# WasifurRahman/BERT_multimodal_transformer

Measured on AMD Instinct MI355X. Metric: train samples/sec MAG-BERT MOSI seq_len=50, higher is better.
Workload: dtype bf16; 1 GPU; MAG-BERT bert-base-uncased, MOSI dims (V=47, A=74), batch 48/GPU, seq_len 50, full optimizer step (fwd+MSE+bwd+HF-AdamW+schedule+zero_grad; inputs resident in HBM), dropout on, random-init weights; global_batch=48, seq_len=50, parallelism=dp1, step_call=mb_bert_train_step, hipGraph replay

## Files before the change

### bert_multimodal_transformer_amd/csrc/engine.hip

```cpp
#include "dp_step.h"

struct LayerOff { size_t wqkv, wo, w1, w2, bqkv, bo, ln1w, ln1b, b1, b2, ln2w, ln2b; };
struct LayerWs { size_t qkv, ctx, s1, st1, y1, u, g, s2, st2, stats; };

struct mb_bert_engine : StepMixin {
    mb_bert_config c;
    std::vector<TensorInfo> tensors;
    std::vector<LayerOff> lo;
    size_t word, pos, type, emb_lnw, emb_lnb, wp, bp, wc, bc;
    size_t mag_whv, mag_wha, mag_wv, mag_wa, mag_bhv, mag_bha, mag_bv, mag_ba, mag_lnw, mag_lnb;
    size_t n_params, n_decay, sh_begin, sh_end;
    size_t n_update_end() const { return n_params; }
    int n_layers() const { return c.num_layers; }
    size_t layer_begin(int l) const { return lo[l].wqkv; }
    size_t layers_end() const { return wp; }
    int width() const { return c.hidden_size; }
    size_t layer_end(int l) const { return l + 1 < c.num_layers ? lo[l + 1].wqkv : wp; }
    bool embed_all_frozen() const { return range_frozen(word, mag_whv) && range_frozen(emb_lnw, bp); }
    WordSkip word_skip(char* w) const {
        if (!(stamp_off != 0 && stamp_enable && idcnt_enable)) return {};
        return WordSkip{stamp_table(w), stamp_state(w), word, word + (size_t)c.vocab_size * c.hidden_size, (uint32_t)c.hidden_size};
    }
    MagWs mw;
    size_t ws_mag, ws_emb, ws_emb_st, ws_head_z, ws_head_pooled, ws_logits;
// ... 6 lines not shown
    size_t ws_ids, ws_seg, ws_mask, ws_labels;
    size_t ws_bytes;
    float* P = nullptr; float* G = nullptr; char* SH = nullptr; char* ws = nullptr;
    const int64_t* ids = nullptr; const int64_t* seg = nullptr; const int64_t* mask = nullptr;
    int B = 0, L = 0, training = 0;
    int padT = -1;
    int prefetch = 1;
    int pf_qkv = 0;
    RideOpts ride_opts;
    int ride_blocks = 0;
    float* ride_m = nullptr; float* ride_v = nullptr;
    size_t ride_cursor = 0;
    long ride_params = 0;
    int group_wgrad = 256;
    bool grouped = false;
    float* attn_out = nullptr;
    const float* head_mask = nullptr;
    const float* emb_in = nullptr;
    const int64_t* pos_ids = nullptr;
    bool ran_forward = false;

    bool ws_zeroed = false;
    uint64_t seed = 0, step = 0;
    float* logits = nullptr;

    size_t add(const std::string& name, std::vector<int64_t> shape, int decay, size_t& cursor) {
        TensorInfo t;
        t.name = name; t.ndim = (int)shape.size(); t.decay = decay; t.numel = 1;
        for (int i = 0; i < 4; ++i) t.shape[i] = i < t.ndim ? shape[i] : 1;
        for (auto s : shape) t.numel *= (size_t)s;
// ... 310 lines not shown
    if (!cfg || !out) return MB_ERR_ARG;
    const int Hc = cfg->hidden_size;
    if ((Hc != 256 && Hc != 512 && Hc != 768 && Hc != 1024) || cfg->num_heads * 64 != Hc || cfg->num_layers < 1) return MB_ERR_SHAPE;
    if (cfg->intermediate_size % 128 || cfg->max_seq < 1 || cfg->max_seq > 512 || cfg->max_batch < 1) return MB_ERR_SHAPE;
    if (cfg->max_seq > cfg->max_position || cfg->num_labels < 1) return MB_ERR_SHAPE;
    if (cfg->dtype != DT_F32 && cfg->dtype != DT_BF16) return MB_ERR_DTYPE;
    mb_bert_engine* e = new mb_bert_engine();
    e->c = *cfg;
    e->read_env();
    e->ride_opts.read_env();
    e->group_wgrad = env_int("MB_GROUP_WGRAD", e->group_wgrad);
    e->ride_blocks = env_int("MB_ADAMW_RIDE_BLOCKS", e->ride_blocks);
    e->ride_params = env_long("MB_ADAMW_RIDE_PARAMS", e->ride_params);
    e->prefetch = env_int("MB_PREFETCH", e->prefetch);
    e->pf_qkv = env_int("MB_PF_QKV", e->pf_qkv);
    if (e->group_wgrad == 256 && (cfg->dtype != DT_BF16 || cfg->hidden_size % 256 != 0 || cfg->intermediate_size % 256 != 0)) e->group_wgrad = 128;
    e->grouped = (e->group_wgrad == 64 || e->group_wgrad == 128 || e->group_wgrad == 256) && cfg->hidden_size % e->group_wgrad == 0 &&
                 cfg->intermediate_size % e->group_wgrad == 0;

    build_layout(e);
    e->ow_covers = e->grouped;
    e->stale_begin = e->lo[0].wqkv; e->stale_end = e->wp;
    *out = e;
    return MB_OK;
}
void mb_bert_destroy(mb_bert_engine* e) {
    if (!e) return;
    e->destroy_prof();
    e->drop_graphs();
    e->free_class_table();
// ... 134 lines not shown
        const bool sh_ok = e->c.dtype != DT_BF16 || (e->sh_begin <= rb && re <= e->sh_end);
        if (take == 0 || rb % 4 || !sh_ok) return r;
        const bool keep = e->keep_in_step() && e->stale_begin <= rb && re <= e->stale_end;
        r = AdamRide{e->P + rb, e->G + rb, e->ride_m + rb, e->ride_v + rb, e->c.dtype == DT_BF16 ? (bf16*)(e->SH + rb * 2) : nullptr,
                     take / 4, dyn, blocks / 8 * 8, keep ? 0 : 1};
        e->ride_cursor = rb;
        return r;
    };
    if (stage_begin < 0) stage_begin = 0;
    if (stage_end > NL + 2) stage_end = NL + 2;
    if (stage_begin == 0) CK(e->begin_backward_pass(e->G, st));
    float* P = e->P; float* G = e->G;
    char* ws = e->ws;
    const bool hd = e->training && c.hidden_dropout > 0.f;
    const GradAcc acc = e->acc_of(ws, G);
    for (int stage = stage_begin; stage < stage_end; ++stage) {
        if (stage == 0) {
            CK(head_backward(dt, dlogits, e->logits, labels, loss_scale, (const float*)(ws + e->ws_head_pooled), P + e->wc,
                             ws + e->ws_dz, G + e->wc, G + e->bc, B, H, c.num_labels, e->key(SITE_HEAD, c.hidden_dropout),
                             st, acc, G + e->bp, ws + e->ws_dxa, (size_t)T * H * esize(dt)));
            const char* xf = ws + e->ws_x[NL];
            CK(gemm(dt, GEMM_TN, EPI_ACCUM_F32, H, H, B, ws + e->ws_dz, H, xf, L * H, nullptr, H, nullptr, G + e->wp, nullptr,
                    nullptr, 0, kNoDrop, 1, 64, st));
            CK(gemm(dt, GEMM_NN, EPI_ADD_RES, B, H, H, ws + e->ws_dz, H, e->W(e->wp), H, ws + e->ws_dxa, L * H, nullptr,
                    nullptr, nullptr, nullptr, 0, kNoDrop, 1, 64, st));
        } else if (stage <= NL) {
            const int l = NL - stage;
            const LayerOff& o = e->lo[l];
            const LayerWs& w = e->lw[l];
            char* dx = ws + e->ws_dxa;
            char* dy1 = ws + e->ws_dxb;
            const int par = l & 1;
            char* dsA = ws + e->ws_ds[par];
            char* dzdA = hd ? ws + e->ws_dzd[par] : dsA;
            char* dsB = ws + e->ws_ds2[par];
            char* dzdB = hd ? ws + e->ws_dzd2[par] : dsB;
            char* du = ws + e->ws_du[par];
            char* dqkv = ws + e->ws_dqkv[par];
            int nblk = 0;
            float* lnp_a = (float*)(ws + e->ws_lnp_a) + (size_t)l * e->lnp_stride;
            float* lnp_b = (float*)(ws + e->ws_lnp_b) + (size_t)l * e->lnp_stride;
            const bool defer_ln = e->in_step && !e->stage_mode && NL + 2 <= MB_LN_MAX_LAYERS;
            CK(ln_backward_partials(dt, dx, ws + w.s2, P + o.ln2w, (const float*)(ws + w.st2), (const float*)(ws + w.st2) + T, dsA,
                                    hd ? dzdA : nullptr, lnp_a, &nblk, T, H, e->key(SITE_LAYER0 + 4 * l + 2, c.hidden_dropout), st,
                                    Prefetch{e->prefetch ? e->W(o.w1) : nullptr, (size_t)2 * I * H * (dt == DT_BF16 ? 2 : 4), nullptr}));
            GemmArgs wg[4] = {wgrad_args(H, I, Tk, dzdA, H, ws + w.g, I, G + o.w2, I),
                              wgrad_args(I, H, Tk, du, I, ws + w.y1, H, G + o.w1, H),
                              wgrad_args(H, H, Tk, dzdB, H, ws + w.ctx, H, G + o.wo, H),
                              wgrad_args(3 * H, H, Tk, dqkv, 3 * H, ws + e->ws_x[l], H, G + o.wqkv, H)};
            const bool grouped = e->grouped;
            const bool wfrozen = e->skipping() && e->unwritten(o.wqkv, e->layer_end(l));
            if (wfrozen) ++e->frz_wgrad_skipped;
            if (grouped)
                for (GemmArgs& a : wg) a.overwrite = e->ow_pass ? 1 : 0;
            auto dgrad_ride = [&](int mode, int Mo, int No, int Ko, const void* dY, int ldy, const void* Wt, int ldw, void* dX, int ldx, const void* R, int ldr,
                                  float* colsum) -> int {
                return dgrad_with_riders(dt, mode, Mo, No, Ko, dY, ldy, Wt, ldw, dX, ldx, R, ldr, colsum, kNoDrop, acc, st, grouped && e->ride_m != nullptr,
// ... 79 lines not shown
                                 G + e->emb_lnb, B, L, H, c.pad_token_id, e->key(SITE_EMB, c.hidden_dropout), st, e->pos_ids, acc,
                                 (float*)(ws + e->ws_lnp_a) + (size_t)(NL + 1) * e->lnp_stride, &eblk,
                                 (float*)(ws + e->ws_lnp_b) + (size_t)(NL + 1) * e->lnp_stride,
                                 (e->in_step && e->counted && e->ids && !e->emb_in) ? (int*)(ws + e->idcnt_off) : nullptr));
            {
                const int first = defer_ln ? 0 : NL;
                LnReduceDst dst = {};
                for (int k = first; k < NL; ++k) {
                    const LayerOff& ok = e->lo[k];
                    float* const d6[6] = {G + ok.ln2w, G + ok.ln2b, G + ok.b2, G + ok.ln1w, G + ok.ln1b, G + ok.bo};
                    for (int q = 0; q < 6; ++q) dst.d[k - first][q] = d6[q];
                }
                float* const m6[6] = {G + e->mag_bhv, G + e->mag_bha, G + e->mag_bv, G + e->mag_ba, G + e->mag_lnw, G + e->mag_lnb};
                for (int q = 0; q < 6; ++q) dst.d[NL - first][q] = m6[q];
                dst.nblk[NL - first] = mblk; dst.nblk[NL + 1 - first] = eblk;
                if (!emb_frozen) { dst.d[NL + 1 - first][0] = G + e->emb_lnw; dst.d[NL + 1 - first][1] = G + e->emb_lnb; }
                if (e->pos_ids == nullptr && !emb_frozen) {
                    dst.d[NL + 1 - first][2] = G + e->type; dst.d[NL + 1 - first][3] = G + e->type + H;
                }
                CK(ln_reduce_partials_layers((const float*)(ws + e->ws_lnp_a) + (size_t)first * e->lnp_stride,
                                             (const float*)(ws + e->ws_lnp_b) + (size_t)first * e->lnp_stride, e->lnp_stride, NL + 2 - first,
                                             e->lnp_nblk, H, dst, st, acc));
            }
            CK(grad_fold(acc, G, e->det_begin, e->det_end, st));
        }
    }
    return MB_OK;
}


static int enqueue_step(mb_bert_engine* e, int B, int L, float* logits, float* loss, float* loss_run, float* m, float* v,
                        float loss_scale, hipStream_t st) {
    char* ws = e->ws;
    const int NL = e->c.num_layers;
    const float* lab = (const float*)(ws + e->ws_in_lab);
    float* keep_attn = e->attn_out;
    e->attn_out = nullptr;
// ... 133 lines not shown
    e->attn_out = nullptr;
    struct Restore { mb_bert_engine* e; float* p; ~Restore() { e->attn_out = p; } } restore{e, keep_attn};
    return e->run_stage_graph(B, L, -1, 0, logits, loss, loss_run, 0.f, mode, st, [&](hipStream_t s) {
        return mb_bert_forward(e, (const int64_t*)(ws + e->ws_in_ids), (const float*)(ws + e->ws_in_vis), (const float*)(ws + e->ws_in_aco),
                               (const int64_t*)(ws + e->ws_in_mask), (const int64_t*)(ws + e->ws_in_seg), (const float*)(ws + e->ws_in_lab), B, L, 1,
                               0, 0, logits, loss, loss_run, s);
    });
}
int mb_bert_stage_backward(mb_bert_engine* e, float loss_scale, int stage, int mode, void* stream) {
    hipStream_t st = (hipStream_t)stream;
    if (!e || !e->G || !e->ran_forward || !e->training) return MB_ERR_ARG;
    if (stage < 0 || stage > e->c.num_layers + 1 || (mode != 1 && mode != 2)) return MB_ERR_ARG;
    if (e->prof) mode = 2;
    if (stage == 0) CK(e->begin_backward_pass(e->G, st));
    const float* lab = (const float*)(e->ws + e->ws_in_lab);
    return e->run_stage_graph(e->B, e->L, stage, e->ow_pass ? 1 : 0, e->logits, nullptr, nullptr, loss_scale, mode, st, [&](hipStream_t s) {
        return mb_bert_backward(e, nullptr, lab, loss_scale, stage, stage + 1, s);
    });
}

const int64_t* mb_bert_staged_input_ids(const mb_bert_engine* e) { return (e && e->ws) ? (const int64_t*)(e->ws + e->ws_in_ids) : nullptr; }

int mb_bert_load_batch(mb_bert_engine* e, const int64_t* input_ids, const float* visual, const float* acoustic,
                       const int64_t* attention_mask, const int64_t* token_type_ids, const float* labels, int B, int L,
                       const void** staged6, void* stream) {
    hipStream_t st = (hipStream_t)stream;
    if (!e || !e->ws || !staged6) return MB_ERR_ARG;
    const mb_bert_config& c = e->c;
    if (B < 1 || B > c.max_batch || L < 1 || L > c.max_seq) return MB_ERR_SHAPE;
    if (!input_ids || !visual || !acoustic || !attention_mask || !token_type_ids) return MB_ERR_ARG;
    const int T = B * L;
// ... 67 lines not shown
    return MB_OK;
}
int mb_bert_set_position_ids(mb_bert_engine* e, const int64_t* position_ids) {
    if (!e) return MB_ERR_ARG;
    e->pos_ids = position_ids;
    return MB_OK;
}
const float* mb_bert_inputs_embeds_grad(const mb_bert_engine* e) {
    if (!e || !e->ws || !e->ran_forward) return nullptr;
    return (const float*)(e->ws + e->ws_dsum);
}
int mb_bert_backward_outputs(mb_bert_engine* e, const void* d_sequence_output, const void* d_pooler_preact, void* stream) {
    hipStream_t st = (hipStream_t)stream;
    if (!e || !e->G || !e->ran_forward) return MB_ERR_ARG;
    CK(e->begin_backward_pass(e->G, st));
    const mb_bert_config& c = e->c;
    const int dt = c.dtype, H = c.hidden_size, B = e->B, L = e->L, T = B * L, NL = c.num_layers;
    char* ws = e->ws;
    const size_t bytes = (size_t)T * H * esize(dt);
    if (d_sequence_output) CK((int)hipMemcpyAsync(ws + e->ws_dxa, d_sequence_output, bytes, hipMemcpyDeviceToDevice, st));
    else CK(zero_fill(ws + e->ws_dxa, bytes, st));
    if (d_pooler_preact) {
        const char* xf = ws + e->ws_x[NL];
        CK(gemm(dt, GEMM_TN, EPI_ACCUM_F32, H, H, B, d_pooler_preact, H, xf, L * H, nullptr, H, nullptr, e->G + e->wp, nullptr, nullptr, 0,
                kNoDrop, 1, 64, st));
        CK(colsum(dt, d_pooler_preact, H, e->G + e->bp, B, H, st, e->acc_of(ws, e->G)));
        CK(gemm(dt, GEMM_NN, EPI_ADD_RES, B, H, H, d_pooler_preact, H, e->W(e->wp), H, ws + e->ws_dxa, L * H, nullptr, nullptr, nullptr,
                ws + e->ws_dxa, L * H, kNoDrop, 1, 64, st));
    }
    return MB_OK;
// ... 31 lines not shown
```

### bert_multimodal_transformer_amd/csrc/engine_common.h

```cpp
#pragma once
#include <string>
#include <vector>
#include <cstring>
#include <cstdio>
#include <cstdlib>
#include <cmath>
#include <algorithm>
#include "kernels.h"
#include "../../include/magbert_hip.h"

using namespace mb;
static_assert(MB_UPDATE_CLASSES_MAX == MB_CLASSES_MAX && MB_UPDATE_SEGMENTS_MAX == MB_SEGMENTS_MAX, "public limits = the kernels' limits");

namespace {

struct TensorInfo {
    std::string name;
    size_t off, numel;
    int ndim;
    int64_t shape[4];
    int decay;
};

inline size_t align_up(size_t x, size_t a) { return (x + a - 1) / a * a; }
// ... 222 lines not shown
            int dev = 0, n = 0;
            if (hipGetDevice(&dev) == hipSuccess && hipDeviceGetAttribute(&n, hipDeviceAttributeMultiprocessorCount, dev) == hipSuccess) cus = n;
            if (cus <= 0) cus = 256;
        }
        return cus;
    }
    bool grads_stale = false, ow_covers = false;
    size_t stale_begin = 0, stale_end = 0;
    int keep_enable = 1;
    bool keep_in_step() const { return keep_enable && ow_enable && ow_covers && stale_end > stale_begin; }
    int materialize_grads(float* G, hipStream_t st) {
        if (grads_stale && G) CK(zero_fill(G + stale_begin, (stale_end - stale_begin) * sizeof(float), st));
        grads_stale = false;
        return MB_OK;
    }
    int begin_backward_pass(float* G, hipStream_t st) {
        if (in_step) return MB_OK;
        stamp_live = word_zero = false;
        frz_dirty = true;
        ow_pass = grads_zero && ow_enable;
        grads_zero = false;
        if (!(ow_pass && ow_covers)) CK(materialize_grads(G, st));
        grads_stale = false;
        return MB_OK;
    }

    bool prof = false;
    std::vector<hipEvent_t> pev;
    int prof_layers = 0;
    int set_profiling(int on, int layers) {
        if (on && pev.empty()) {
// ... 583 lines not shown
```

### bert_multimodal_transformer_amd/csrc/gemm.hip

```cpp
#include "gemm_tile.h"
#include "adamw_dev.h"

namespace mb {

constexpr int PITCH = 144;

template <class T, int BROWS, bool KMAJ>
struct Stager {
    static constexpr int EPV = 16 / sizeof(T);
    static constexpr int BKE = 128 / sizeof(T);
    static constexpr int NREG = BROWS / 8;
    uint32_t r[NREG];

    __device__ __forceinline__ void load(const T* __restrict__ base, int ld, int row0, int nrows, int k0, int kend, int tid) {
        if constexpr (!KMAJ) {
#pragma unroll
            for (int i = 0; i < BROWS / 32; ++i) {
                const int rr = (tid >> 3) + 32 * i, c = tid & 7;
                const int g = row0 + rr;
                u32x4 v = {0u, 0u, 0u, 0u};
                if (g < nrows) v = *(const u32x4*)(base + (size_t)g * ld + k0 + c * EPV);
                r[4 * i + 0] = v[0]; r[4 * i + 1] = v[1]; r[4 * i + 2] = v[2]; r[4 * i + 3] = v[3];
            }
        } else {
// ... 593 lines not shown
        }
        return launch_cfg<T, 128, 128, AK, BK, MODE>(a, splits, st);
    } else
    if (v2ok) {
        int ns = 2, kb = 128;
        if (env.stages > 0) { kb = (env.stages / 10 == 2) ? 64 : 128; ns = env.stages % 10; }
        if (kb == 64 && (p.kchunk % (64 / (int)sizeof(T)) != 0)) kb = 128;
        if (sizeof(T) == 2 && ns <= 2 && p.kchunk / (kb / (int)sizeof(T)) < 2) ns = 3;
#define MB_LAUNCH2(NS, KBV) MB_GEMM_LAUNCH((gemm2_kernel<T, BM, BN, AK, BK, MODE, NS, KBV>), grid, dim3(256), st, p, &p, 1)
        if constexpr (BM == 64 && BN == 64 && sizeof(T) == 2) {
            if (env.ksplit && env.stages <= 0 && p.kchunk % 128 == 0 && p.kchunk >= 1024 && splits == 1 && tiles <= 512) {
                MB_GEMM_LAUNCH((gemm2_kernel<T, BM, BN, AK, BK, MODE, 2, 256, true>), grid, dim3(256), st, p, &p, 1);
                return (int)hipGetLastError();
            }
            if (env.stages64 >= 3 && env.stages <= 0 && splits == 1 && p.kchunk / BKE >= 2 && tiles <= 512) ns = env.stages64 > 4 ? 4 : env.stages64;
        }
        if (kb == 128) {
            if (BM == 128) { if (ns <= 2) MB_LAUNCH2(2, 128); else if (ns == 3) MB_LAUNCH2(3, 128); else MB_LAUNCH2(4, 128); }
            else { if (ns <= 2) MB_LAUNCH2(2, 128); else if (ns == 3) MB_LAUNCH2(3, 128); else MB_LAUNCH2(4, 128); }
        } else {
            if (ns <= 3) MB_LAUNCH2(3, 64); else if (ns == 4) MB_LAUNCH2(4, 64); else MB_LAUNCH2(5, 64);
        }
#undef MB_LAUNCH2
    } else {
        MB_GEMM_LAUNCH((gemm_kernel<T, BM, BN, AK, BK, MODE>), grid, dim3(256), st, p, &p, 1);
    }
    return (int)hipGetLastError();
}

static int tile_n768() { return host_env().tile_n768; }
// ... 242 lines not shown
```

### bert_multimodal_transformer_amd/csrc/gemm_tile.h

```cpp
#pragma once
#include <cstdlib>
#include <algorithm>
#include <type_traits>
#include "kernels.h"

namespace mb {

template <int BM, int BN>
__device__ __forceinline__ bool tile_origin(const GemmArgs& p, int& m0, int& n0, int bid = blockIdx.x) {
    const int xcd = bid & 7, j = bid >> 3;
    const int xm = xcd / p.reg_n, xn = xcd % p.reg_n;
    const int tm = xm * p.tpr_m + j / p.tpr_n, tn = xn * p.tpr_n + j % p.tpr_n;
    m0 = tm * BM;
    n0 = tn * BN;
    return m0 < p.M && n0 < p.N && (j / p.tpr_n) < p.tpr_m;
}

template <int BM, int BN>
__device__ __forceinline__ bool grouped_tile_origin(const GroupedGemmArgs& ga, int& g, int& m0, int& n0) {
    const int bid = (int)blockIdx.x - ga.ride.blocks;
    g = 0;
    if (ga.chunk > 0) {
        const int xcd = bid & 7, j = bid >> 3;
        const int lin = xcd * ga.chunk + j;
// ... 48 lines not shown
    static __device__ __forceinline__ void store(float* p, const float (&v)[8]) {
        *(f32x4*)p = f32x4{v[0], v[1], v[2], v[3]};
        *(f32x4*)(p + 4) = f32x4{v[4], v[5], v[6], v[7]};
    }
};

template <class T, int BM, int BN, int MODE, int NW>
struct EpiPre {
    static constexpr int TPR = BN / 8;
    static constexpr int RPP = NW * 64 / TPR;
    static constexpr int NR = BM / RPP;
    static constexpr bool HAS_R = sizeof(T) == 2 && (MODE == EPI_BIAS_DROP_RES || MODE == EPI_ADD_RES || MODE == EPI_DGELU);
    bf16x8 r[HAS_R ? NR : 1];
    float bias8[8];
    DropKey key;
    int ldc, cvalid, overwrite;
    __device__ __forceinline__ void fetch(const GemmArgs& p, int m0, int n0, int tid) {
        ldc = p.ldc; cvalid = p.cvalid; overwrite = p.overwrite;
        asm volatile("" : "+s"(ldc), "+s"(cvalid), "+s"(overwrite));
        key = p.drop;
        key.resolve();
        const int n = n0 + (tid % TPR) * 8;
#pragma unroll
        for (int q = 0; q < 8; ++q) bias8[q] = 0.f;
        if constexpr (MODE == EPI_BIAS || MODE == EPI_BIAS_F32 || MODE == EPI_BIAS_GELU || MODE == EPI_BIAS_DROP_RES) {
            if (p.bias && n < p.N) Vec8<float>::load(p.bias + n, bias8);
        }
        if constexpr (HAS_R) {
#pragma unroll
            for (int it = 0; it < NR; ++it) {
                const int m = m0 + tid / TPR + it * RPP;
                r[it] = bf16x8{};
                if (p.R && m < p.M && n < p.N) r[it] = *(const bf16x8*)((const bf16*)p.R + (size_t)m * p.ldr + n);
            }
// ... 76 lines not shown
            if constexpr (Pre::HAS_R) {
#pragma unroll
                for (int q = 0; q < 8; ++q) res[q] = (float)pre.r[it][q];
            } else {
                if (p.R) Vec8<T>::load((const T*)p.R + (size_t)m * p.ldr + n, res);
            }
        }
        const size_t off = (size_t)m * pre.ldc + n;
        if constexpr (MODE == EPI_BIAS || MODE == EPI_BIAS_F32) {
#pragma unroll
            for (int q = 0; q < 8; ++q) v[q] = v[q] * p.alpha + bias8[q];
            if constexpr (MODE == EPI_BIAS) Vec8<T>::store(C + off, v);
            else Vec8<float>::store(p.Cf + off, v);
        } else if constexpr (MODE == EPI_BIAS_GELU) {
            float g[8];
            const uint32_t gidx = (uint32_t)m * (uint32_t)p.N + (uint32_t)n;
#pragma unroll
            for (int q = 0; q < 8; q += 2) {
                const f32x2 u = {v[q] + bias8[q], v[q + 1] + bias8[q + 1]};
                f32x2 gg, dg;
                gelu_pair(u, gg, dg);
                g[q] = gg.x;
                g[q + 1] = gg.y;
                v[q] = dg.x;
                v[q + 1] = dg.y;
            }
            if (dkey.thresh != 0u) {
#pragma unroll
                for (int q = 0; q < 8; ++q) g[q] *= drop_mult(dkey, gidx + q);
            }
            Vec8<T>::store(C + off, v);
            Vec8<T>::store((T*)p.C2 + off, g);
        } else if constexpr (MODE == EPI_BIAS_DROP_RES) {
            const uint32_t idx = (uint32_t)m * (uint32_t)p.N + (uint32_t)n;
#pragma unroll
            for (int q = 0; q < 8; ++q) v[q] = (v[q] + bias8[q]) * drop_mult(dkey, idx + q) + res[q];
            Vec8<T>::store(C + off, v);
        } else if constexpr (MODE == EPI_ADD_RES) {
#pragma unroll
            for (int q = 0; q < 8; ++q) v[q] += res[q];
            Vec8<T>::store(C + off, v);
        } else if constexpr (MODE == EPI_DGELU) {
            const uint32_t gidx = (uint32_t)m * (uint32_t)p.N + (uint32_t)n;
#pragma unroll
            for (int q = 0; q < 8; ++q) { v[q] *= res[q] * drop_mult(dkey, gidx + q); cs[q] += v[q]; }
            Vec8<T>::store(C + off, v);
        } else if constexpr (MODE == EPI_ACCUM_F32) {
            float* dst = p.Cf + off;
            if (gridDim.y > 1) {
#pragma unroll
                for (int q = 0; q < 8; ++q) atomicAdd(dst + q, v[q]);
            } else if (pre.overwrite) {
                Vec8<float>::store(dst, v);
            } else {
                float o[8];
                Vec8<float>::load(dst, o);
#pragma unroll
                for (int q = 0; q < 8; ++q) o[q] += v[q];
// ... 218 lines not shown
```

### bert_multimodal_transformer_amd/csrc/kernels.h

```cpp
#pragma once
#include <cstdio>
#include <cstdlib>
#include "common.h"

namespace mb {

enum {
    MB_OK = 0,
    MB_ERR_SHAPE = 1001,
    MB_ERR_MODE = 1002,
    MB_ERR_DTYPE = 1003,
    MB_ERR_ARG = 1004,
    MB_ERR_COMM = 1005,
};

inline void ck_trace(const char* expr, const char* file, int line, int code) {
    static int on = -1;
    if (on < 0) { const char* v = getenv("MB_CK_TRACE"); on = (v && atoi(v)) ? 1 : 0; }
    if (on) fprintf(stderr, "[magbert] %s:%d: %s -> %d\n", file, line, expr, code);
}

enum { GEMM_NT = 0,
       GEMM_NN = 1,
       GEMM_TN = 2 };
// ... 16 lines not shown
    int M, N, K, lda, ldb;
    void* C; int ldc;
    void* C2;
    float* Cf;
    const float* bias;
    float* colsum;
    const void* R; int ldr;
    float alpha;
    DropKey drop;
    int kchunk;
    int dbg;
    int reg_m, reg_n, tpr_m, tpr_n;
    int overwrite;
    int cvalid;
    unsigned long long* trace;
    int bseg; size_t bseg_stride;
    GradAcc acc;
};
int gemm_trace_fetch(unsigned long long* host_out, int max_blocks);

int gemm_launch(int dtype, int layout, int mode, const GemmArgs& a, int splits, int tile, hipStream_t st);

#define MB_MAX_GROUP 8
struct AdamRide {
    float *p, *g, *m, *v;
    bf16* shadow;
    size_t n4;
    const AdamArgs* dyn;
    int blocks;
    int zero_grad;
};
// ... 7 lines not shown
};
int gemm_nn_ride_tiles(int dtype, int mode, const GemmArgs& a, int* per_cu);
int gemm_nn_ride_launch(int dtype, int mode, const GemmArgs& a, const AdamRide& ride, hipStream_t st);
int gemm_grouped_tn_ok(int dtype, const GemmArgs* probs, int count, int tile);
int gemm_grouped_tn_launch(int dtype, const GemmArgs* probs, int count, int tile, hipStream_t st, int stages = 0,
                           const AdamRide* ride = nullptr);

int ln_forward(int dtype, const void* x, const float* gamma, const float* beta, float eps, void* y,
               float* mean, float* rstd, int rows, int H, DropKey drop, hipStream_t st,
               Prefetch pf = {nullptr, 0, nullptr});
int ln_backward(int dtype, const void* dy, const void* x, const float* gamma, const float* mean, const float* rstd,
                void* dx, void* dx_drop, float* dgamma, float* dbeta, float* dbias,
                int rows, int H, DropKey drop_out, DropKey drop_in, hipStream_t st);
int grad_fold(GradAcc acc, float* g, size_t begin, size_t end, hipStream_t st);
size_t ln_partials_floats(int rows, int H);
int ln_backward_partials(int dtype, const void* dy, const void* x, const float* gamma, const float* mean, const float* rstd,
                         void* dx, void* dx_drop, float* partials, int* nblk, int rows, int H, DropKey drop_in, hipStream_t st,
                         Prefetch pf = {nullptr, 0, nullptr});
int ln_reduce_partials(const float* partials_a, const float* partials_b, int nblk, int H, float* const* dst6, hipStream_t st, GradAcc acc = {});
#define MB_LN_MAX_LAYERS 32
struct LnReduceDst { float* d[MB_LN_MAX_LAYERS][6]; int nblk[MB_LN_MAX_LAYERS]; };
int ln_reduce_partials_layers(const float* partials_a, const float* partials_b, size_t layer_stride, int layers, int nblk, int H,
                              const LnReduceDst& dst, hipStream_t st, GradAcc acc = {});

int embed_ln_forward(int dtype, const int64_t* ids, const int64_t* seg, const float* word, const float* pos,
                     const float* type, const float* gamma, const float* beta, float eps, void* out,
                     float* mean, float* rstd, int B, int L, int H, DropKey drop, hipStream_t st,
                     const int64_t* pos_ids = nullptr);
int embed_ln_backward(int dtype, const void* dout, const int64_t* ids, const int64_t* seg, const float* word,
                      const float* pos, const float* type, const float* gamma, const float* mean, const float* rstd,
                      float* dsum_ws, float* dword, float* dpos, float* dtype_, float* dgamma, float* dbeta,
                      int B, int L, int H, int pad_id, DropKey drop, hipStream_t st, const int64_t* pos_ids = nullptr, GradAcc acc = {},
                      float* part = nullptr, int* nblk = nullptr,
// ... 137 lines not shown
```

### bert_multimodal_transformer_amd/csrc/rowops.hip

```cpp
#include <algorithm>
#include "kernels.h"
#include "mag_pack.h"

namespace mb {

template <int CH>
struct RowStat {
    static __device__ __forceinline__ void compute(const f32x4 (&v)[CH], float eps, float& mu, float& rs) {
        constexpr float invH = 1.0f / (CH * 256);
        float s = 0.f;
#pragma unroll
        for (int c = 0; c < CH; ++c) s += (v[c][0] + v[c][1]) + (v[c][2] + v[c][3]);
        mu = wave_sum(s) * invH;
        float q = 0.f;
#pragma unroll
        for (int c = 0; c < CH; ++c) {
#pragma unroll
            for (int r = 0; r < 4; ++r) { const float d = v[c][r] - mu; q += d * d; }
        }
        rs = 1.0f / sqrtf(wave_sum(q) * invH + eps);
    }
};

template <class T, int CH>
// ... 46 lines not shown
    const int lane = threadIdx.x & 63, wave = threadIdx.x >> 6;
#pragma unroll
    for (int q = 0; q < NQ; ++q)
#pragma unroll
        for (int c = 0; c < CH; ++c) *(f32x4*)(lds + (wave * NQ + q) * H + (c * 64 + lane) * 4) = part[q][c];
    __syncthreads();
    for (int i = threadIdx.x; i < NQ * H; i += 256) {
        const int q = i / H, col = i % H;
        if (dst[q] == nullptr) continue;
        const float s = lds[(0 * NQ + q) * H + col] + lds[(1 * NQ + q) * H + col] + lds[(2 * NQ + q) * H + col] +
                        lds[(3 * NQ + q) * H + col];
        grad_add(acc, dst[q] + col, s);
    }
}

template <class T, int CH, int RPW, bool PARTIAL, int NWV = 4>
__global__ void __launch_bounds__(NWV * 64) ln_bwd_kernel(const T* __restrict__ dy, const T* __restrict__ x,
                                                     const float* __restrict__ gamma, const float* __restrict__ mean,
                                                     const float* __restrict__ rstd, T* __restrict__ dx,
                                                     T* __restrict__ dx_drop, float* dgamma, float* dbeta, float* dbias,
                                                     int rows, DropKey drop_out, DropKey drop_in, Prefetch pf) {
    drop_out.resolve();
    drop_in.resolve();
    constexpr int H = CH * 256;
    constexpr float invH = 1.0f / H;
    constexpr int SL = NWV > 8 ? 8 : NWV;
    __shared__ float lds[SL * 3 * H];
    const int lane = threadIdx.x & 63, wave = threadIdx.x >> 6;
    f32x4 part[3][CH];
#pragma unroll
    for (int q = 0; q < 3; ++q)
#pragma unroll
        for (int c = 0; c < CH; ++c) part[q][c] = f32x4{0.f, 0.f, 0.f, 0.f};
    f32x4 g[CH];
#pragma unroll
    for (int c = 0; c < CH; ++c) g[c] = *(const f32x4*)(gamma + (c * 64 + lane) * 4);
    for (int i = 0; i < RPW; ++i) {
        const int row = (blockIdx.x * NWV + wave) * RPW + i;
        if (row >= rows) break;
        const float mu = mean[row], rs = rstd[row];
        f32x4 dyv[CH], xh[CH];
        float s1 = 0.f, s2 = 0.f;
#pragma unroll
        for (int c = 0; c < CH; ++c) {
            const int col = (c * 64 + lane) * 4;
            dyv[c] = load4(dy + (size_t)row * H + col);
            const uint32_t idx = (uint32_t)row * H + col;
#pragma unroll
            for (int r = 0; r < 4; ++r) dyv[c][r] *= drop_mult(drop_out, idx + r);
            xh[c] = (load4(x + (size_t)row * H + col) - mu) * rs;
            const f32x4 dxh = dyv[c] * g[c];
            s1 += (dxh[0] + dxh[1]) + (dxh[2] + dxh[3]);
            const f32x4 t = dxh * xh[c];
            s2 += (t[0] + t[1]) + (t[2] + t[3]);
        }
        const float m1 = wave_sum(s1) * invH, m2 = wave_sum(s2) * invH;
#pragma unroll
        for (int c = 0; c < CH; ++c) {
            const int col = (c * 64 + lane) * 4;
            f32x4 d = (dyv[c] * g[c] - m1 - xh[c] * m2) * rs;
            store4(dx + (size_t)row * H + col, d);
            part[0][c] += dyv[c] * xh[c];
            part[1][c] += dyv[c];
            if (dx_drop) {
                const uint32_t idx = (uint32_t)row * H + col;
#pragma unroll
                for (int r = 0; r < 4; ++r) d[r] *= drop_mult(drop_in, idx + r);
                store4(dx_drop + (size_t)row * H + col, d);
            }
            part[2][c] += d;
        }
    }
    u32x4 pfv[8];
    prefetch_issue<8>(pf, gamma, pfv);
    if constexpr (PARTIAL) {
        if constexpr (NWV > SL) {
            if (wave >= SL) {
#pragma unroll
                for (int q = 0; q < 3; ++q)
#pragma unroll
                    for (int c = 0; c < CH; ++c) *(f32x4*)(lds + ((wave - SL) * 3 + q) * H + (c * 64 + lane) * 4) = part[q][c];
            }
            __syncthreads();
// ... 368 lines not shown
    MB_DISPATCH_T(dtype, MB_DISPATCH_CH(H, {
        hipLaunchKernelGGL((ln_fwd_kernel<T, CH>), dim3((rows + 3) / 4), dim3(256), 0, st, (const T*)x, gamma, beta, eps,
                           (T*)y, mean, rstd, rows, drop, pf);
    }))
    return (int)hipGetLastError();
}

int ln_backward(int dtype, const void* dy, const void* x, const float* gamma, const float* mean, const float* rstd,
                void* dx, void* dx_drop, float* dgamma, float* dbeta, float* dbias, int rows, int H, DropKey drop_out,
                DropKey drop_in, hipStream_t st) {
    if (rows <= 0) return MB_OK;
    constexpr int RPW = 4;
    MB_DISPATCH_T(dtype, MB_DISPATCH_CH(H, {
        hipLaunchKernelGGL((ln_bwd_kernel<T, CH, RPW, false>), dim3((rows + 4 * RPW - 1) / (4 * RPW)), dim3(256), 0, st,
                           (const T*)dy, (const T*)x, gamma, mean, rstd, (T*)dx, (T*)dx_drop, dgamma, dbeta, dbias, rows,
                           drop_out, drop_in, Prefetch{nullptr, 0, nullptr});
    }))
    return (int)hipGetLastError();
}

size_t ln_partials_floats(int rows, int H) { return (size_t)((rows + 4 * LN_RPW - 1) / (4 * LN_RPW)) * 3 * H; }

constexpr int LN_NWV = MB_LN_NWV;
int ln_backward_partials(int dtype, const void* dy, const void* x, const float* gamma, const float* mean, const float* rstd,
                         void* dx, void* dx_drop, float* partials, int* nblk, int rows, int H, DropKey drop_in,
                         hipStream_t st, Prefetch pf) {
    if (rows <= 0) { *nblk = 0; return MB_OK; }
    const int nb = (rows + LN_NWV * LN_RPW - 1) / (LN_NWV * LN_RPW);
    *nblk = nb;
    const DropKey nodrop = {0u, 0u, 0u, 1.0f};
    MB_DISPATCH_T(dtype, MB_DISPATCH_CH(H, {
        hipLaunchKernelGGL((ln_bwd_kernel<T, CH, LN_RPW, true, LN_NWV>), dim3(nb), dim3(LN_NWV * 64), 0, st, (const T*)dy, (const T*)x, gamma,
                           mean, rstd, (T*)dx, (T*)dx_drop, partials, (float*)nullptr, (float*)nullptr, rows, nodrop, drop_in, pf);
    }))
    return (int)hipGetLastError();
}

int ln_reduce_partials(const float* pa, const float* pb, int nblk, int H, float* const* d, hipStream_t st, GradAcc acc) {
    if (nblk <= 0) return MB_OK;
    hipLaunchKernelGGL(ln_reduce_kernel, dim3((H + 63) / 64, 6, 8), dim3(256), 0, st, pa, pb, nblk, H, d[0], d[1], d[2], d[3], d[4],
                       d[5], acc);
    return (int)hipGetLastError();
}

int ln_reduce_partials_layers(const float* pa, const float* pb, size_t layer_stride, int layers, int nblk, int H,
                              const LnReduceDst& dst, hipStream_t st, GradAcc acc) {
    if (nblk <= 0 || layers <= 0) return MB_OK;
    if (layers > MB_LN_MAX_LAYERS) return MB_ERR_SHAPE;
// ... 284 lines not shown
```

Before: 15370 samples/s.

## Backprop top encoder layer FFN and output projection only through CLS rows

The pooler uses only the CLS token, so in the top layer the gradient is nonzero only on CLS rows through LN2, the FFN, LN1 and the attention output projection. The new path runs those LN backward passes and GEMMs on B rows instead of B*L, using strided row access and a rowmul factor so dropout indices still match. It then runs full attention backward and the QKV weight gradient as before. It also adds a 4-stage pipeline choice for rowmul GEMMs with long K, and adds complexity around zeroing the dx workspace and deferring the LN partial reduction.

```diff
diff --git a/bert_multimodal_transformer_amd/csrc/engine.hip b/bert_multimodal_transformer_amd/csrc/engine.hip
--- a/bert_multimodal_transformer_amd/csrc/engine.hip
+++ b/bert_multimodal_transformer_amd/csrc/engine.hip
@@ -44,6 +44,8 @@
     long ride_params = 0;
     int group_wgrad = 256;
     bool grouped = false;
+    int top_cls = 1, top_wtile = 64, top_qkv_tile = 64;
+    int top_nblk = 0;
     float* attn_out = nullptr;
     const float* head_mask = nullptr;
     const float* emb_in = nullptr;
@@ -384,6 +386,9 @@
     e->ride_params = env_long("MB_ADAMW_RIDE_PARAMS", e->ride_params);
     e->prefetch = env_int("MB_PREFETCH", e->prefetch);
     e->pf_qkv = env_int("MB_PF_QKV", e->pf_qkv);
+    e->top_cls = env_int("MB_TOP_CLS", e->top_cls);
+    e->top_wtile = env_int("MB_TOP_CLS_WTILE", e->top_wtile) == 128 ? 128 : 64;
+    e->top_qkv_tile = env_int("MB_TOP_CLS_QKV_TILE", e->top_qkv_tile);
     if (e->group_wgrad == 256 && (cfg->dtype != DT_BF16 || cfg->hidden_size % 256 != 0 || cfg->intermediate_size % 256 != 0)) e->group_wgrad = 128;
     e->grouped = (e->group_wgrad == 64 || e->group_wgrad == 128 || e->group_wgrad == 256) && cfg->hidden_size % e->group_wgrad == 0 &&
                  cfg->intermediate_size % e->group_wgrad == 0;
@@ -548,16 +553,19 @@
     char* ws = e->ws;
     const bool hd = e->training && c.hidden_dropout > 0.f;
     const GradAcc acc = e->acc_of(ws, G);
+    const bool top_short = e->top_cls && e->grouped;
     for (int stage = stage_begin; stage < stage_end; ++stage) {
         if (stage == 0) {
             CK(head_backward(dt, dlogits, e->logits, labels, loss_scale, (const float*)(ws + e->ws_head_pooled), P + e->wc,
                              ws + e->ws_dz, G + e->wc, G + e->bc, B, H, c.num_labels, e->key(SITE_HEAD, c.hidden_dropout),
-                             st, acc, G + e->bp, ws + e->ws_dxa, (size_t)T * H * esize(dt)));
+                             st, acc, G + e->bp, ws + e->ws_dxa,
+                             (top_short ? e->ws_dxb - e->ws_dxa : (size_t)0) + (size_t)T * H * esize(dt)));
             const char* xf = ws + e->ws_x[NL];
             CK(gemm(dt, GEMM_TN, EPI_ACCUM_F32, H, H, B, ws + e->ws_dz, H, xf, L * H, nullptr, H, nullptr, G + e->wp, nullptr,
                     nullptr, 0, kNoDrop, 1, 64, st));
             CK(gemm(dt, GEMM_NN, EPI_ADD_RES, B, H, H, ws + e->ws_dz, H, e->W(e->wp), H, ws + e->ws_dxa, L * H, nullptr,
                     nullptr, nullptr, nullptr, 0, kNoDrop, 1, 64, st));
+            e->cls_rows = true;
         } else if (stage <= NL) {
             const int l = NL - stage;
             const LayerOff& o = e->lo[l];
@@ -575,6 +583,64 @@
             float* lnp_a = (float*)(ws + e->ws_lnp_a) + (size_t)l * e->lnp_stride;
             float* lnp_b = (float*)(ws + e->ws_lnp_b) + (size_t)l * e->lnp_stride;
             const bool defer_ln = e->in_step && !e->stage_mode && NL + 2 <= MB_LN_MAX_LAYERS;
+            if (l == NL - 1) e->top_nblk = 0;
+            if (l == NL - 1 && top_short && e->cls_rows) {
+                const int LH = L * H, LI = L * I;
+                char* dyc = ws + e->ws_ds2[par];
+                char* dctx = ws + e->ws_dxb;
+                const char* dzdBp = hd ? dzdB : dx;
+                const int dzdB_ld = hd ? H : LH;
+                const float* st2 = (const float*)(ws + w.st2); const float* st1 = (const float*)(ws + w.st1);
+                auto sgemm = [&](int layout, int mode, int Mo, int No, int Ko, const void* A, int lda, const void* Bm, int ldb, void* C, int ldc,
+                                 float* colsum, const void* R, int ldr) -> int {
+                    GemmArgs a = {};
+                    a.A = A; a.B = Bm; a.M = Mo; a.N = No; a.K = Ko; a.lda = lda; a.ldb = ldb; a.C = C; a.ldc = ldc; a.R = R; a.ldr = ldr;
+                    a.alpha = 1.0f; a.drop = kNoDrop; a.kchunk = Ko; a.colsum = colsum; a.acc = acc; a.rowmul = L;
+                    return gemm_launch(dt, layout, mode, a, 1, 64, st);
+                };
+                int nb = 0, nb1 = 0;
+                LnRows r2; r2.dy = L; r2.tr = L;
+                CK(ln_backward_partials(dt, dx, ws + w.s2, P + o.ln2w, st2, st2 + T, dsA, hd ? dzdA : nullptr, lnp_a, &nb, B, H,
+                                        e->key(SITE_LAYER0 + 4 * l + 2, c.hidden_dropout), st, Prefetch{nullptr, 0, nullptr}, r2));
+                CK(sgemm(GEMM_NN, EPI_DGELU, B, I, H, dzdA, H, e->W(o.w2), I, du, I, G + o.b1, ws + w.u, LI));
+                CK(sgemm(GEMM_NN, EPI_ADD_RES, B, H, I, du, I, e->W(o.w1), H, dyc, H, nullptr, dsA, H));
+                LnRows r1; r1.dx = L; r1.tr = L;
+                CK(ln_backward_partials(dt, dyc, ws + w.s1, P + o.ln1w, st1, st1 + T, dx, hd ? dzdB : nullptr, lnp_b, &nb1, B, H,
+                                        e->key(SITE_LAYER0 + 4 * l + 1, c.hidden_dropout), st, Prefetch{nullptr, 0, nullptr}, r1));
+                e->top_nblk = nb;
+                const bool defer_top = e->in_step && !e->stage_mode && NL + 2 <= MB_LN_MAX_LAYERS;
+                if (!defer_top) {
+                    float* const dst6[6] = {G + o.ln2w, G + o.ln2b, G + o.b2, G + o.ln1w, G + o.ln1b, G + o.bo};
+                    CK(ln_reduce_partials(lnp_a, lnp_b, nb, H, dst6, st, acc));
+                }
+                CK(sgemm(GEMM_NN, EPI_ADD_RES, B, H, H, dzdBp, dzdB_ld, e->W(o.wo), H, dctx, LH, nullptr, nullptr, 0));
+                CK(attention_backward(dt, ws + w.qkv, e->mask, ws + w.ctx, dctx, dqkv, G + o.bqkv, B, L, nh,
+                                      e->key(SITE_LAYER0 + 4 * l + 0, c.attn_dropout), st,
+                                      e->head_mask ? e->head_mask + (size_t)l * nh : nullptr, acc, nullptr, e->attn_stats(w)));
+                const bool wfrozen = e->skipping() && e->unwritten(o.wqkv, e->layer_end(l));
+                if (wfrozen) ++e->frz_wgrad_skipped;
+                if (e->prof) CK((int)hipEventRecord(e->pev[2 * l], st));
+                if (!wfrozen) {
+                    GemmArgs ws3[3] = {wgrad_args(H, I, B, dzdA, H, ws + w.g, LI, G + o.w2, I),
+                                       wgrad_args(I, H, B, du, I, ws + w.y1, LH, G + o.w1, H),
+                                       wgrad_args(H, H, B, dzdBp, dzdB_ld, ws + w.ctx, LH, G + o.wo, H)};
+                    for (GemmArgs& a : ws3) {
+                        a.overwrite = e->ow_pass ? 1 : 0;
+                        CK(gemm_launch(dt, GEMM_TN, EPI_ACCUM_F32, a, 1, e->top_wtile, st));
+                    }
+                    GemmArgs wq = wgrad_args(3 * H, H, Tk, dqkv, 3 * H, ws + e->ws_x[l], H, G + o.wqkv, H);
+                    wq.overwrite = e->ow_pass ? 1 : 0;
+                    int qt = e->top_qkv_tile > 0 ? e->top_qkv_tile : e->group_wgrad;
+                    if (!gemm_grouped_tn_ok(dt, &wq, 1, qt)) qt = e->group_wgrad;
+                    if (qt == 256 && !gemm_grouped_tn_ok(dt, &wq, 1, 256)) qt = 128;
+                    if (!gemm_grouped_tn_ok(dt, &wq, 1, qt)) return MB_ERR_SHAPE;
+                    CK(gemm_grouped_tn_launch(dt, &wq, 1, qt, st));
+                }
+                if (e->prof) CK((int)hipEventRecord(e->pev[2 * l + 1], st));
+                CK(gemm(dt, GEMM_NN, EPI_ADD_RES, T, H, 3 * H, dqkv, 3 * H, e->W(o.wqkv), H, dx, H, nullptr, nullptr, nullptr, dx, H, kNoDrop, 1, 0, st));
+                (void)nb1;
+                continue;
+            }
             CK(ln_backward_partials(dt, dx, ws + w.s2, P + o.ln2w, (const float*)(ws + w.st2), (const float*)(ws + w.st2) + T, dsA,
                                     hd ? dzdA : nullptr, lnp_a, &nblk, T, H, e->key(SITE_LAYER0 + 4 * l + 2, c.hidden_dropout), st,
                                     Prefetch{e->prefetch ? e->W(o.w1) : nullptr, (size_t)2 * I * H * (dt == DT_BF16 ? 2 : 4), nullptr}));
@@ -684,13 +750,14 @@
                 float* const m6[6] = {G + e->mag_bhv, G + e->mag_bha, G + e->mag_bv, G + e->mag_ba, G + e->mag_lnw, G + e->mag_lnb};
                 for (int q = 0; q < 6; ++q) dst.d[NL - first][q] = m6[q];
                 dst.nblk[NL - first] = mblk; dst.nblk[NL + 1 - first] = eblk;
+                if (first == 0 && e->top_nblk > 0) dst.nblk[NL - 1] = e->top_nblk;
                 if (!emb_frozen) { dst.d[NL + 1 - first][0] = G + e->emb_lnw; dst.d[NL + 1 - first][1] = G + e->emb_lnb; }
                 if (e->pos_ids == nullptr && !emb_frozen) {
                     dst.d[NL + 1 - first][2] = G + e->type; dst.d[NL + 1 - first][3] = G + e->type + H;
                 }
                 CK(ln_reduce_partials_layers((const float*)(ws + e->ws_lnp_a) + (size_t)first * e->lnp_stride,
                                              (const float*)(ws + e->ws_lnp_b) + (size_t)first * e->lnp_stride, e->lnp_stride, NL + 2 - first,
-                                             e->lnp_nblk, H, dst, st, acc));
+                                             e->lnp_nblk > 0 ? e->lnp_nblk : 1, H, dst, st, acc));
             }
             CK(grad_fold(acc, G, e->det_begin, e->det_end, st));
         }
@@ -854,7 +921,8 @@
     if (e->prof) mode = 2;
     if (stage == 0) CK(e->begin_backward_pass(e->G, st));
     const float* lab = (const float*)(e->ws + e->ws_in_lab);
-    return e->run_stage_graph(e->B, e->L, stage, e->ow_pass ? 1 : 0, e->logits, nullptr, nullptr, loss_scale, mode, st, [&](hipStream_t s) {
+    struct HeadDone { mb_bert_engine* e; bool on; ~HeadDone() { if (on) e->cls_rows = true; } } head_done{e, stage == 0};
+    return e->run_stage_graph(e->B, e->L, stage, (e->ow_pass ? 1 : 0) | (e->cls_rows ? 2 : 0), e->logits, nullptr, nullptr, loss_scale, mode, st, [&](hipStream_t s) {
         return mb_bert_backward(e, nullptr, lab, loss_scale, stage, stage + 1, s);
     });
 }
@@ -952,6 +1020,7 @@
     hipStream_t st = (hipStream_t)stream;
     if (!e || !e->G || !e->ran_forward) return MB_ERR_ARG;
     CK(e->begin_backward_pass(e->G, st));
+    e->cls_rows = false;
     const mb_bert_config& c = e->c;
     const int dt = c.dtype, H = c.hidden_size, B = e->B, L = e->L, T = B * L, NL = c.num_layers;
     char* ws = e->ws;
diff --git a/bert_multimodal_transformer_amd/csrc/engine_common.h b/bert_multimodal_transformer_amd/csrc/engine_common.h
--- a/bert_multimodal_transformer_amd/csrc/engine_common.h
+++ b/bert_multimodal_transformer_amd/csrc/engine_common.h
@@ -260,7 +260,9 @@
         grads_stale = false;
         return MB_OK;
     }
+    bool cls_rows = false;
     int begin_backward_pass(float* G, hipStream_t st) {
+        cls_rows = false;
         if (in_step) return MB_OK;
         stamp_live = word_zero = false;
         frz_dirty = true;
diff --git a/bert_multimodal_transformer_amd/csrc/gemm.hip b/bert_multimodal_transformer_amd/csrc/gemm.hip
--- a/bert_multimodal_transformer_amd/csrc/gemm.hip
+++ b/bert_multimodal_transformer_amd/csrc/gemm.hip
@@ -631,6 +631,7 @@
                 return (int)hipGetLastError();
             }
             if (env.stages64 >= 3 && env.stages <= 0 && splits == 1 && p.kchunk / BKE >= 2 && tiles <= 512) ns = env.stages64 > 4 ? 4 : env.stages64;
+            if (p.rowmul > 1 && env.stages <= 0 && splits == 1 && p.kchunk / BKE >= 16 && ns == 3) ns = 4;
         }
         if (kb == 128) {
             if (BM == 128) { if (ns <= 2) MB_LAUNCH2(2, 128); else if (ns == 3) MB_LAUNCH2(3, 128); else MB_LAUNCH2(4, 128); }
diff --git a/bert_multimodal_transformer_amd/csrc/gemm_tile.h b/bert_multimodal_transformer_amd/csrc/gemm_tile.h
--- a/bert_multimodal_transformer_amd/csrc/gemm_tile.h
+++ b/bert_multimodal_transformer_amd/csrc/gemm_tile.h
@@ -86,10 +86,10 @@
     bf16x8 r[HAS_R ? NR : 1];
     float bias8[8];
     DropKey key;
-    int ldc, cvalid, overwrite;
+    int ldc, cvalid, overwrite, rowmul;
     __device__ __forceinline__ void fetch(const GemmArgs& p, int m0, int n0, int tid) {
-        ldc = p.ldc; cvalid = p.cvalid; overwrite = p.overwrite;
-        asm volatile("" : "+s"(ldc), "+s"(cvalid), "+s"(overwrite));
+        ldc = p.ldc; cvalid = p.cvalid; overwrite = p.overwrite; rowmul = p.rowmul > 1 ? p.rowmul : 1;
+        asm volatile("" : "+s"(ldc), "+s"(cvalid), "+s"(overwrite), "+s"(rowmul));
         key = p.drop;
         key.resolve();
         const int n = n0 + (tid % TPR) * 8;
@@ -196,7 +196,7 @@
             else Vec8<float>::store(p.Cf + off, v);
         } else if constexpr (MODE == EPI_BIAS_GELU) {
             float g[8];
-            const uint32_t gidx = (uint32_t)m * (uint32_t)p.N + (uint32_t)n;
+            const uint32_t gidx = (uint32_t)m * (uint32_t)pre.rowmul * (uint32_t)p.N + (uint32_t)n;
 #pragma unroll
             for (int q = 0; q < 8; q += 2) {
                 const f32x2 u = {v[q] + bias8[q], v[q + 1] + bias8[q + 1]};
@@ -214,7 +214,7 @@
             Vec8<T>::store(C + off, v);
             Vec8<T>::store((T*)p.C2 + off, g);
         } else if constexpr (MODE == EPI_BIAS_DROP_RES) {
-            const uint32_t idx = (uint32_t)m * (uint32_t)p.N + (uint32_t)n;
+            const uint32_t idx = (uint32_t)m * (uint32_t)pre.rowmul * (uint32_t)p.N + (uint32_t)n;
 #pragma unroll
             for (int q = 0; q < 8; ++q) v[q] = (v[q] + bias8[q]) * drop_mult(dkey, idx + q) + res[q];
             Vec8<T>::store(C + off, v);
@@ -223,7 +223,7 @@
             for (int q = 0; q < 8; ++q) v[q] += res[q];
             Vec8<T>::store(C + off, v);
         } else if constexpr (MODE == EPI_DGELU) {
-            const uint32_t gidx = (uint32_t)m * (uint32_t)p.N + (uint32_t)n;
+            const uint32_t gidx = (uint32_t)m * (uint32_t)pre.rowmul * (uint32_t)p.N + (uint32_t)n;
 #pragma unroll
             for (int q = 0; q < 8; ++q) { v[q] *= res[q] * drop_mult(dkey, gidx + q); cs[q] += v[q]; }
             Vec8<T>::store(C + off, v);
diff --git a/bert_multimodal_transformer_amd/csrc/kernels.h b/bert_multimodal_transformer_amd/csrc/kernels.h
--- a/bert_multimodal_transformer_amd/csrc/kernels.h
+++ b/bert_multimodal_transformer_amd/csrc/kernels.h
@@ -54,7 +54,9 @@
     int overwrite;
     int cvalid;
     unsigned long long* trace;
-    int bseg; size_t bseg_stride;
+    int bseg;
+    int rowmul;
+    size_t bseg_stride;
     GradAcc acc;
 };
 int gemm_trace_fetch(unsigned long long* host_out, int max_blocks);
@@ -92,9 +94,10 @@
                 int rows, int H, DropKey drop_out, DropKey drop_in, hipStream_t st);
 int grad_fold(GradAcc acc, float* g, size_t begin, size_t end, hipStream_t st);
 size_t ln_partials_floats(int rows, int H);
+struct LnRows { int dy = 1, dx = 1, dxd = 1, tr = 1; };
 int ln_backward_partials(int dtype, const void* dy, const void* x, const float* gamma, const float* mean, const float* rstd,
                          void* dx, void* dx_drop, float* partials, int* nblk, int rows, int H, DropKey drop_in, hipStream_t st,
-                         Prefetch pf = {nullptr, 0, nullptr});
+                         Prefetch pf = {nullptr, 0, nullptr}, LnRows rm = {});
 int ln_reduce_partials(const float* partials_a, const float* partials_b, int nblk, int H, float* const* dst6, hipStream_t st, GradAcc acc = {});
 #define MB_LN_MAX_LAYERS 32
 struct LnReduceDst { float* d[MB_LN_MAX_LAYERS][6]; int nblk[MB_LN_MAX_LAYERS]; };
diff --git a/bert_multimodal_transformer_amd/csrc/rowops.hip b/bert_multimodal_transformer_amd/csrc/rowops.hip
--- a/bert_multimodal_transformer_amd/csrc/rowops.hip
+++ b/bert_multimodal_transformer_amd/csrc/rowops.hip
@@ -84,14 +84,15 @@
     }
 }
 
-template <class T, int CH, int RPW, bool PARTIAL, int NWV = 4>
+template <class T, int CH, int RPW, bool PARTIAL, int NWV = 4, bool STRIDED = false>
 __global__ void __launch_bounds__(NWV * 64) ln_bwd_kernel(const T* __restrict__ dy, const T* __restrict__ x,
                                                      const float* __restrict__ gamma, const float* __restrict__ mean,
                                                      const float* __restrict__ rstd, T* __restrict__ dx,
                                                      T* __restrict__ dx_drop, float* dgamma, float* dbeta, float* dbias,
-                                                     int rows, DropKey drop_out, DropKey drop_in, Prefetch pf) {
+                                                     int rows, DropKey drop_out, DropKey drop_in, Prefetch pf, LnRows rm) {
     drop_out.resolve();
     drop_in.resolve();
+    if constexpr (!STRIDED) rm = LnRows{};
     constexpr int H = CH * 256;
     constexpr float invH = 1.0f / H;
     constexpr int SL = NWV > 8 ? 8 : NWV;
@@ -108,17 +109,18 @@
     for (int i = 0; i < RPW; ++i) {
         const int row = (blockIdx.x * NWV + wave) * RPW + i;
         if (row >= rows) break;
-        const float mu = mean[row], rs = rstd[row];
+        const size_t tr = (size_t)row * rm.tr;
+        const float mu = mean[tr], rs = rstd[tr];
         f32x4 dyv[CH], xh[CH];
         float s1 = 0.f, s2 = 0.f;
 #pragma unroll
         for (int c = 0; c < CH; ++c) {
             const int col = (c * 64 + lane) * 4;
-            dyv[c] = load4(dy + (size_t)row * H + col);
-            const uint32_t idx = (uint32_t)row * H + col;
+            dyv[c] = load4(dy + (size_t)row * rm.dy * H + col);
+            const uint32_t idx = (uint32_t)tr * H + col;
 #pragma unroll
             for (int r = 0; r < 4; ++r) dyv[c][r] *= drop_mult(drop_out, idx + r);
-            xh[c] = (load4(x + (size_t)row * H + col) - mu) * rs;
+            xh[c] = (load4(x + tr * H + col) - mu) * rs;
             const f32x4 dxh = dyv[c] * g[c];
             s1 += (dxh[0] + dxh[1]) + (dxh[2] + dxh[3]);
             const f32x4 t = dxh * xh[c];
@@ -129,14 +131,14 @@
         for (int c = 0; c < CH; ++c) {
             const int col = (c * 64 + lane) * 4;
             f32x4 d = (dyv[c] * g[c] - m1 - xh[c] * m2) * rs;
-            store4(dx + (size_t)row * H + col, d);
+            store4(dx + (size_t)row * rm.dx * H + col, d);
             part[0][c] += dyv[c] * xh[c];
             part[1][c] += dyv[c];
             if (dx_drop) {
-                const uint32_t idx = (uint32_t)row * H + col;
+                const uint32_t idx = (uint32_t)tr * H + col;
 #pragma unroll
                 for (int r = 0; r < 4; ++r) d[r] *= drop_mult(drop_in, idx + r);
-                store4(dx_drop + (size_t)row * H + col, d);
+                store4(dx_drop + (size_t)row * rm.dxd * H + col, d);
             }
             part[2][c] += d;
         }
@@ -535,7 +537,7 @@
     MB_DISPATCH_T(dtype, MB_DISPATCH_CH(H, {
         hipLaunchKernelGGL((ln_bwd_kernel<T, CH, RPW, false>), dim3((rows + 4 * RPW - 1) / (4 * RPW)), dim3(256), 0, st,
                            (const T*)dy, (const T*)x, gamma, mean, rstd, (T*)dx, (T*)dx_drop, dgamma, dbeta, dbias, rows,
-                           drop_out, drop_in, Prefetch{nullptr, 0, nullptr});
+                           drop_out, drop_in, Prefetch{nullptr, 0, nullptr}, LnRows{});
     }))
     return (int)hipGetLastError();
 }
@@ -545,14 +547,18 @@
 constexpr int LN_NWV = MB_LN_NWV;
 int ln_backward_partials(int dtype, const void* dy, const void* x, const float* gamma, const float* mean, const float* rstd,
                          void* dx, void* dx_drop, float* partials, int* nblk, int rows, int H, DropKey drop_in,
-                         hipStream_t st, Prefetch pf) {
+                         hipStream_t st, Prefetch pf, LnRows rm) {
     if (rows <= 0) { *nblk = 0; return MB_OK; }
     const int nb = (rows + LN_NWV * LN_RPW - 1) / (LN_NWV * LN_RPW);
     *nblk = nb;
     const DropKey nodrop = {0u, 0u, 0u, 1.0f};
     MB_DISPATCH_T(dtype, MB_DISPATCH_CH(H, {
-        hipLaunchKernelGGL((ln_bwd_kernel<T, CH, LN_RPW, true, LN_NWV>), dim3(nb), dim3(LN_NWV * 64), 0, st, (const T*)dy, (const T*)x, gamma,
-                           mean, rstd, (T*)dx, (T*)dx_drop, partials, (float*)nullptr, (float*)nullptr, rows, nodrop, drop_in, pf);
+        if (rm.dy != 1 || rm.dx != 1 || rm.dxd != 1 || rm.tr != 1)
+            hipLaunchKernelGGL((ln_bwd_kernel<T, CH, LN_RPW, true, LN_NWV, true>), dim3(nb), dim3(LN_NWV * 64), 0, st, (const T*)dy, (const T*)x, gamma,
+                               mean, rstd, (T*)dx, (T*)dx_drop, partials, (float*)nullptr, (float*)nullptr, rows, nodrop, drop_in, pf, rm);
+        else
+            hipLaunchKernelGGL((ln_bwd_kernel<T, CH, LN_RPW, true, LN_NWV>), dim3(nb), dim3(LN_NWV * 64), 0, st, (const T*)dy, (const T*)x, gamma,
+                               mean, rstd, (T*)dx, (T*)dx_drop, partials, (float*)nullptr, (float*)nullptr, rows, nodrop, drop_in, pf, rm);
     }))
     return (int)hipGetLastError();
 }
```

Result: no change. 15370 samples/s (-0.0%).
